# lucidrains/magvit2-pytorch

Hardware: NVIDIA H100
Metric: video-frames/sec tokenize+decode, 17x128x128 bf16 (higher is better)
Workload: dtype bf16

## Files before the change

### magvit2_pytorch_b200/csrc/tc_common.cuh

```cuda
#pragma once
#include "common.cuh"
#include <cuda.h>
#include <mutex>

namespace mv2 {


__device__ __forceinline__ uint32_t smem_u32(const void* p) { return (uint32_t)__cvta_generic_to_shared(p); }

__device__ __forceinline__ void mbar_init(uint32_t bar, uint32_t count) {
  asm volatile("mbarrier.init.shared::cta.b64 [%0], %1;" ::"r"(bar), "r"(count));
}
__device__ __forceinline__ void mbar_expect_tx(uint32_t bar, uint32_t bytes) {
  asm volatile("mbarrier.arrive.expect_tx.shared::cta.b64 _, [%0], %1;" ::"r"(bar), "r"(bytes) : "memory");
}
__device__ __forceinline__ void mbar_wait(uint32_t bar, uint32_t parity) {
  asm volatile(
      "{\n\t"
      ".reg .pred P1;\n\t"
      "WAIT_LOOP:\n\t"
      "mbarrier.try_wait.parity.shared::cta.b64 P1, [%0], %1, 0x989680;\n\t"
      "@P1 bra DONE;\n\t"
      "bra WAIT_LOOP;\n\t"
      "DONE:\n\t"
      "}" ::"r"(bar), "r"(parity) : "memory");
}
__device__ __forceinline__ void fence_barrier_init() { asm volatile("fence.mbarrier_init.release.cluster;" ::: "memory"); }
__device__ __forceinline__ void fence_proxy_async() { asm volatile("fence.proxy.async.shared::cta;" ::: "memory"); }

__device__ __forceinline__ void tma_load_5d(uint32_t dst, const CUtensorMap* map, uint32_t bar, int c0, int c1, int c2,
                                            int c3, int c4) {
  asm volatile(
      "cp.async.bulk.tensor.5d.shared::cluster.global.tile.mbarrier::complete_tx::bytes [%0], [%1, {%3, %4, %5, %6, %7}], [%2];"
      ::"r"(dst), "l"(map), "r"(bar), "r"(c0), "r"(c1), "r"(c2), "r"(c3), "r"(c4) : "memory");
}
__device__ __forceinline__ void tma_load_2d(uint32_t dst, const CUtensorMap* map, uint32_t bar, int c0, int c1) {
  asm volatile(
      "cp.async.bulk.tensor.2d.shared::cluster.global.tile.mbarrier::complete_tx::bytes [%0], [%1, {%3, %4}], [%2];"
      ::"r"(dst), "l"(map), "r"(bar), "r"(c0), "r"(c1) : "memory");
}
__device__ __forceinline__ void tma_load_3d(uint32_t dst, const CUtensorMap* map, uint32_t bar, int c0, int c1, int c2) {
  asm volatile(
      "cp.async.bulk.tensor.3d.shared::cluster.global.tile.mbarrier::complete_tx::bytes [%0], [%1, {%3, %4, %5}], [%2];"
      ::"r"(dst), "l"(map), "r"(bar), "r"(c0), "r"(c1), "r"(c2) : "memory");
}
__device__ __forceinline__ void tma_prefetch_desc(const CUtensorMap* map) {
  asm volatile("prefetch.tensormap [%0];" ::"l"(map) : "memory");
}

__device__ __forceinline__ void wgmma_fence() { asm volatile("wgmma.fence.sync.aligned;" ::: "memory"); }
__device__ __forceinline__ void wgmma_commit() { asm volatile("wgmma.commit_group.sync.aligned;" ::: "memory"); }
__device__ __forceinline__ void wgmma_wait_all() { asm volatile("wgmma.wait_group.sync.aligned 0;" ::: "memory"); }
template <int N> __device__ __forceinline__ void wgmma_bf16(float (&d)[N / 2], uint64_t da, uint64_t db, uint32_t scale_d);
template <> __device__ __forceinline__ void wgmma_bf16<32>(float (&d)[16], uint64_t da, uint64_t db, uint32_t scale_d) {
  asm volatile(
      "{\n\t.reg .pred p;\n\tsetp.ne.b32 p, %18, 0;\n\t"
      "wgmma.mma_async.sync.aligned.m64n32k16.f32.bf16.bf16 {%0, %1, %2, %3, %4, %5, %6, %7, %8, %9, %10, %11, %12, %13, %14, %15}, %16, %17, p, 1, 1, 0, 0;\n\t}"
      : "+f"(d[0]), "+f"(d[1]), "+f"(d[2]), "+f"(d[3]), "+f"(d[4]), "+f"(d[5]), "+f"(d[6]), "+f"(d[7]), "+f"(d[8]), "+f"(d[9]), "+f"(d[10]), "+f"(d[11]), "+f"(d[12]), "+f"(d[13]), "+f"(d[14]), "+f"(d[15])
      : "l"(da), "l"(db), "r"(scale_d));
}
template <> __device__ __forceinline__ void wgmma_bf16<64>(float (&d)[32], uint64_t da, uint64_t db, uint32_t scale_d) {
  asm volatile(
      "{\n\t.reg .pred p;\n\tsetp.ne.b32 p, %34, 0;\n\t"
      "wgmma.mma_async.sync.aligned.m64n64k16.f32.bf16.bf16 {%0, %1, %2, %3, %4, %5, %6, %7, %8, %9, %10, %11, %12, %13, %14, %15, %16, %17, %18, %19, %20, %21, %22, %23, %24, %25, %26, %27, %28, %29, %30, %31}, %32, %33, p, 1, 1, 0, 0;\n\t}"
      : "+f"(d[0]), "+f"(d[1]), "+f"(d[2]), "+f"(d[3]), "+f"(d[4]), "+f"(d[5]), "+f"(d[6]), "+f"(d[7]), "+f"(d[8]), "+f"(d[9]), "+f"(d[10]), "+f"(d[11]), "+f"(d[12]), "+f"(d[13]), "+f"(d[14]), "+f"(d[15]), "+f"(d[16]), "+f"(d[17]), "+f"(d[18]), "+f"(d[19]), "+f"(d[20]), "+f"(d[21]), "+f"(d[22]), "+f"(d[23]), "+f"(d[24]), "+f"(d[25]), "+f"(d[26]), "+f"(d[27]), "+f"(d[28]), "+f"(d[29]), "+f"(d[30]), "+f"(d[31])
      : "l"(da), "l"(db), "r"(scale_d));
}
template <> __device__ __forceinline__ void wgmma_bf16<128>(float (&d)[64], uint64_t da, uint64_t db, uint32_t scale_d) {
  asm volatile(
      "{\n\t.reg .pred p;\n\tsetp.ne.b32 p, %66, 0;\n\t"
      "wgmma.mma_async.sync.aligned.m64n128k16.f32.bf16.bf16 {%0, %1, %2, %3, %4, %5, %6, %7, %8, %9, %10, %11, %12, %13, %14, %15, %16, %17, %18, %19, %20, %21, %22, %23, %24, %25, %26, %27, %28, %29, %30, %31, %32, %33, %34, %35, %36, %37, %38, %39, %40, %41, %42, %43, %44, %45, %46, %47, %48, %49, %50, %51, %52, %53, %54, %55, %56, %57, %58, %59, %60, %61, %62, %63}, %64, %65, p, 1, 1, 0, 0;\n\t}"
      : "+f"(d[0]), "+f"(d[1]), "+f"(d[2]), "+f"(d[3]), "+f"(d[4]), "+f"(d[5]), "+f"(d[6]), "+f"(d[7]), "+f"(d[8]), "+f"(d[9]), "+f"(d[10]), "+f"(d[11]), "+f"(d[12]), "+f"(d[13]), "+f"(d[14]), "+f"(d[15]), "+f"(d[16]), "+f"(d[17]), "+f"(d[18]), "+f"(d[19]), "+f"(d[20]), "+f"(d[21]), "+f"(d[22]), "+f"(d[23]), "+f"(d[24]), "+f"(d[25]), "+f"(d[26]), "+f"(d[27]), "+f"(d[28]), "+f"(d[29]), "+f"(d[30]), "+f"(d[31]), "+f"(d[32]), "+f"(d[33]), "+f"(d[34]), "+f"(d[35]), "+f"(d[36]), "+f"(d[37]), "+f"(d[38]), "+f"(d[39]), "+f"(d[40]), "+f"(d[41]), "+f"(d[42]), "+f"(d[43]), "+f"(d[44]), "+f"(d[45]), "+f"(d[46]), "+f"(d[47]), "+f"(d[48]), "+f"(d[49]), "+f"(d[50]), "+f"(d[51]), "+f"(d[52]), "+f"(d[53]), "+f"(d[54]), "+f"(d[55]), "+f"(d[56]), "+f"(d[57]), "+f"(d[58]), "+f"(d[59]), "+f"(d[60]), "+f"(d[61]), "+f"(d[62]), "+f"(d[63])
      : "l"(da), "l"(db), "r"(scale_d));
}

__host__ __device__ __forceinline__ uint64_t gmma_desc_hi(uint32_t sbo, uint32_t row_bytes) {
  const uint64_t layout = row_bytes == 128 ? 1 : (row_bytes == 64 ? 2 : 3);
  return ((uint64_t)1 << 16) | ((uint64_t)(sbo >> 4) << 32) | (layout << 62);
}
__device__ __forceinline__ uint32_t desc_lo(uint32_t saddr) { return (saddr & 0x3FFFF) >> 4; }

template <int N> __device__ __forceinline__ void stage_acc(const float (&d)[N / 2], float* stg, int t) {
  const int r = 16 * (t >> 5) + ((t & 31) >> 2), c = 2 * (t & 3);
#pragma unroll
  for (int j = 0; j < N / 8; ++j) {
    *reinterpret_cast<float2*>(stg + r * (N + 4) + 8 * j + c) = make_float2(d[4 * j], d[4 * j + 1]);
    *reinterpret_cast<float2*>(stg + (r + 8) * (N + 4) + 8 * j + c) = make_float2(d[4 * j + 2], d[4 * j + 3]);
  }
}
__device__ __forceinline__ void load_row32(const float* src, int ncols, uint32_t (&r)[32]) {
#pragma unroll
  for (int g = 0; g < 8; ++g) {
    if (g * 4 >= ncols) break;
    const float4 v = *reinterpret_cast<const float4*>(src + 4 * g);
    r[4 * g] = __float_as_uint(v.x); r[4 * g + 1] = __float_as_uint(v.y);
    r[4 * g + 2] = __float_as_uint(v.z); r[4 * g + 3] = __float_as_uint(v.w);
  }
}
__device__ __forceinline__ void named_bar_sync(uint32_t id, uint32_t nthreads) {
  asm volatile("bar.sync %0, %1;" ::"r"(id), "r"(nthreads) : "memory");
}
__device__ __forceinline__ void mbar_arrive(uint32_t bar) {
  asm volatile("mbarrier.arrive.shared::cta.b64 _, [%0];" ::"r"(bar) : "memory");
}

__device__ __forceinline__ uint32_t pack_bf16x2(float a, float b) {
  __nv_bfloat162 v = __floats2bfloat162_rn(a, b);
  return *reinterpret_cast<uint32_t*>(&v);
}



struct TcEpi {
  const float* bias;
  const __nv_bfloat16* res;
  __nv_bfloat16* y;
  int act, shuffle, mode;
  int Co;
  int To, Ho, Wo;
  int out_cf;
  const float* oscale;
};

__device__ __forceinline__ void store8_bf16(__nv_bfloat16* dst, const float (&v)[8]) {
  uint4 o;
  o.x = pack_bf16x2(v[0], v[1]); o.y = pack_bf16x2(v[2], v[3]);
  o.z = pack_bf16x2(v[4], v[5]); o.w = pack_bf16x2(v[6], v[7]);
  *reinterpret_cast<uint4*>(dst) = o;
}

enum { EPI_PLAIN = 0, EPI_GEGLU = 1, EPI_SHUFFLE = 2, EPI_RAGGED = 3, EPI_PLAIN_RES = 4, EPI_FUSED_RU = 5, EPI_SHUFFLE_ST = 6,
       EPI_DOWN_SPACE = 7 };

__device__ __forceinline__ float ex2_approx(float x) {
  float y;
// ... 211 lines not shown
```

### magvit2_pytorch_b200/csrc/tc_conv.cu

```cuda
#include "common.cuh"
#include "tc_common.cuh"
#include <cuda.h>
#include <mutex>
#include <algorithm>
#include <string.h>

namespace mv2 {

constexpr int TC_MAX_TAPS = 64;
constexpr int TC_MAX_MAPS = 8;
constexpr int TC_BM = 128;

struct alignas(64) TcParams {
  CUtensorMap amap[TC_MAX_MAPS];
  CUtensorMap wmap;
  int8_t tap_map[TC_MAX_TAPS], tap_dt[TC_MAX_TAPS], tap_dh[TC_MAX_TAPS], tap_dw[TC_MAX_TAPS];
  int ntaps, kchunks, ci_pad, bk;
  int B, To, Ho, Wo, Co;
  int bt, bh, bw, tt, th, tw;
  int bn, stages;
  TcEpi epi;
};

template <int MODE, int BN>
__global__ void __launch_bounds__(384, 1) tc_conv_kernel(const __grid_constant__ TcParams p) {
  extern __shared__ uint8_t smem_raw[];
  const uint32_t smem_base = (smem_u32(smem_raw) + 1023u) & ~1023u;
  const int warp = threadIdx.x >> 5, lane = threadIdx.x & 31;
  const int bk = p.bk;
  const uint32_t row_bytes = bk * 2;
  const uint32_t a_bytes = TC_BM * row_bytes;
  const uint32_t b_bytes = BN * row_bytes;
  const uint32_t stage_bytes = a_bytes + b_bytes;
  const uint32_t bar_base = smem_base + p.stages * stage_bytes;
  const uint32_t full0 = bar_base, empty0 = bar_base + 8 * p.stages;
  const uint32_t sbias_u = (empty0 + 8 * p.stages + 15) & ~15u;
  float* sbias = reinterpret_cast<float*>(smem_raw + (sbias_u - smem_u32(smem_raw)));
  float* stg_all = sbias + BN;

  int tile = blockIdx.x;
  const int iw = tile % p.tw; tile /= p.tw;
  const int ih = tile % p.th; tile /= p.th;
  const int it = tile % p.tt; tile /= p.tt;
  const int b = tile;
  const int w0 = iw * p.bw, h0 = ih * p.bh, t0 = it * p.bt;
  const int n0 = blockIdx.y * BN;

  if (threadIdx.x == 0) {
    for (int s = 0; s < p.stages; ++s) {
      mbar_init(full0 + 8 * s, 1);
      mbar_init(empty0 + 8 * s, 8);
    }
    fence_barrier_init();
  }
  if (warp == 0 && lane == 0) {
    tma_prefetch_desc(&p.wmap);
    tma_prefetch_desc(&p.amap[0]);
  }
  if (warp >= 4)
    for (int i = threadIdx.x - 128; i < BN; i += 256) sbias[i] = (p.epi.bias && n0 + i < p.Co) ? p.epi.bias[n0 + i] : 0.f;
  __syncthreads();
  pdl_wait();
  pdl_launch_dependents();

  const int n_iters = p.ntaps * p.kchunks;
  if (warp == 0) {
    if (lane == 0) {
      uint32_t s = 0, ph = 0;
      int tap = 0, kc = 0;
      for (int i = 0; i < n_iters; ++i) {
        mbar_wait(empty0 + 8 * s, ph ^ 1);
        mbar_expect_tx(full0 + 8 * s, stage_bytes);
        const uint32_t sa = smem_base + s * stage_bytes;
        tma_load_5d(sa, &p.amap[p.tap_map[tap]], full0 + 8 * s, kc * bk, w0 + p.tap_dw[tap], h0 + p.tap_dh[tap],
                    t0 + p.tap_dt[tap], b);
        tma_load_2d(sa + a_bytes, &p.wmap, full0 + 8 * s, tap * p.ci_pad + kc * bk, n0);
        if (++kc == p.kchunks) { kc = 0; ++tap; }
        if (++s == (uint32_t)p.stages) { s = 0; ph ^= 1; }
      }
    }
  } else if (warp >= 4) {
    const int wg = (warp - 4) >> 2, t = threadIdx.x & 127;
    const uint64_t d_hi = gmma_desc_hi(8 * row_bytes, row_bytes);
    const int ksteps = bk >> 4;
    const uint32_t stage16 = stage_bytes >> 4, a16 = a_bytes >> 4, wg16 = (uint32_t)wg * ((64 * row_bytes) >> 4);
    uint32_t s = 0, ph = 0, lo = desc_lo(smem_base);
    float acc[BN / 2];
    for (int i = 0; i < n_iters; ++i) {
      mbar_wait(full0 + 8 * s, ph);
      wgmma_fence();
      const uint64_t ad = d_hi | (uint64_t)(lo + wg16);
      const uint64_t bd = d_hi | (uint64_t)(lo + a16);
      wgmma_bf16<BN>(acc, ad, bd, i > 0 ? 1u : 0u);
      if (ksteps > 1) wgmma_bf16<BN>(acc, ad + 2, bd + 2, 1u);
      if (ksteps > 2) {
        wgmma_bf16<BN>(acc, ad + 4, bd + 4, 1u);
        wgmma_bf16<BN>(acc, ad + 6, bd + 6, 1u);
      }
      wgmma_commit();
      wgmma_wait_all();
      __syncwarp();
      if (lane == 0) mbar_arrive(empty0 + 8 * s);
      if (++s == (uint32_t)p.stages) { s = 0; ph ^= 1; lo = desc_lo(smem_base); } else { lo += stage16; }
    }
    float* stg = stg_all + wg * 64 * (BN + 4);
    stage_acc<BN>(acc, stg, t);
    named_bar_sync(1 + wg, 128);
    const int wq = warp & 3;
    const int sub = 2 * wg + (wq & 1), half = wq >> 1;
    const int row = sub * 32 + lane;
    const int lw = row % p.bw, lh = (row / p.bw) % p.bh, lt = row / (p.bw * p.bh);
    const int wo = w0 + lw, ho = h0 + lh, to = t0 + lt;
    const bool row_ok = wo < p.Wo && ho < p.Ho && to < p.To;
    const int64_t row_base = ((((int64_t)b * p.To + to) * p.Ho + ho) * p.Wo + wo) * p.Co;
    const float* srow = stg + (row - 64 * wg) * (BN + 4);
    for (int c0 = half * 32; c0 < BN; c0 += 64) {
      uint32_t r[32];
      load_row32(srow + c0, 32, r);
      if (row_ok) epi_chunk32<MODE>(p.epi, r, 32, n0 + c0, sbias + c0, b, to, ho, wo, row_base);
    }
  }
}

#define MV2_TC_BN(M) {tc_conv_kernel<M, 32>, tc_conv_kernel<M, 64>, tc_conv_kernel<M, 128>}
static void (*const g_tc_kernels[3][3])(TcParams) = {MV2_TC_BN(EPI_RAGGED), MV2_TC_BN(EPI_GEGLU), MV2_TC_BN(EPI_SHUFFLE)};
#undef MV2_TC_BN

}

using namespace mv2;

extern "C" {

int mv2_tc_conv_supported(const mv2_tc_conv_args* a) {
  if (!a) return 0;
  if (a->Ci % 16 != 0) return 0;
  if (a->kt * a->kh * a->kw > TC_MAX_TAPS) return 0;
  if (a->st < 1 || a->st > 2 || a->sh < 1 || a->sh > 2 || a->sw < 1 || a->sw > 2) return 0;
  if (a->shuffle != MV2_SHUFFLE_NONE && ((a->shuffle == MV2_SHUFFLE_SPACE ? a->Co / 4 : a->Co / 2) % 8 != 0)) return 0;
  if (a->res && a->Co % 8 != 0) return 0;
  if (a->epi_mode == 1 && (a->Co % 32 != 0 || a->shuffle != MV2_SHUFFLE_NONE || a->res)) return 0;
  if (a->epi_mode == 2 && (!a->res || a->shuffle != MV2_SHUFFLE_NONE)) return 0;
  if (a->epi_mode < 0 || a->epi_mode > 2) return 0;
  if (a->out_layout != 0) return 0;
  if (a->oscale && (a->epi_mode != 0 || a->shuffle != MV2_SHUFFLE_NONE)) return 0;
  return 1;
}

int mv2_tc_conv_forward(const mv2_tc_conv_args* a, void* stream) {
  MV2_CHECK_ARG(a && a->x && a->w && a->y);
  if (!mv2_tc_conv_supported(a)) { set_error("mv2_tc_conv_forward: unsupported shape (Ci=%d Co=%d)", a->Ci, a->Co); return MV2_E_UNSUPPORTED; }

  TcParams p;
  memset(&p, 0, sizeof(p));
  const int bk = (a->Ci % 64 == 0) ? 64 : ((a->Ci % 32 == 0) ? 32 : 16);
  const CUtensorMapSwizzle swz = swizzle_of_row(bk * 2);
  p.bk = bk;
  p.ci_pad = a->Ci;
  p.kchunks = a->Ci / bk;
  p.B = a->B; p.To = a->To; p.Ho = a->Ho; p.Wo = a->Wo; p.Co = a->Co;
  p.bw = std::min(128, pow2_ceil(a->Wo));
  p.bh = std::min(128 / p.bw, pow2_ceil(a->Ho));
  p.bt = 128 / (p.bw * p.bh);
  p.tw = ceil_div(a->Wo, p.bw); p.th = ceil_div(a->Ho, p.bh); p.tt = ceil_div(a->To, p.bt);
  const int bn = a->Co <= 32 ? 32 : (a->Co <= 64 ? 64 : 128);
  const int row_bytes = bk * 2;
  p.bn = bn;
  const int stage_bytes = TC_BM * row_bytes + bn * row_bytes;
  MV2_CHECK_ARG((TC_BM * row_bytes) % 1024 == 0 && (bn * row_bytes) % 1024 == 0);
  const int stg_bytes = 2 * 64 * (bn + 4) * 4;
  int stages = (200 * 1024 - stg_bytes) / stage_bytes;
  stages = std::max(2, std::min(stages, 8));
  stages = std::max(1, std::min(stages, a->kt * a->kh * a->kw * (a->Ci / bk)));
  p.stages = stages;
  p.epi = tc_epi_of(a);

  const int st = a->st, sh = a->sh, sw = a->sw;
  const int nmaps = st * sh * sw;
  MV2_CHECK_ARG(nmaps <= TC_MAX_MAPS);
  const int64_t C = a->Ci, W = a->Wi, H = a->Hi, T = a->Ti;
  for (int pt = 0; pt < st; ++pt)
    for (int ph = 0; ph < sh; ++ph)
      for (int pw = 0; pw < sw; ++pw) {
        const int id = (pt * sh + ph) * sw + pw;
        const int64_t nW = (W - pw + sw - 1) / sw, nH = (H - ph + sh - 1) / sh, nT = (T - pt + st - 1) / st;
        if (nW <= 0 || nH <= 0 || nT <= 0) { set_error("empty stride phase (dimension smaller than stride)"); return MV2_E_UNSUPPORTED; }
        const cuuint64_t dims[5] = {(cuuint64_t)C, (cuuint64_t)nW, (cuuint64_t)nH, (cuuint64_t)nT, (cuuint64_t)a->B};
// ... 46 lines not shown
```

### magvit2_pytorch_b200/csrc/tc_slab.cu

```cuda
#include "common.cuh"
#include "tc_common.cuh"
#include <cuda.h>
#include <algorithm>
#include <mutex>
#include <map>
#include <vector>
#include <string.h>

namespace mv2 {

struct alignas(64) SlabParams {
  CUtensorMap amap;
  CUtensorMap wmap;
  CUtensorMap wmap2;
  int kt, kh, kw, pt, ph, pw;
  int st;
  int Ci, kchunks, row_bytes;
  int B, T, H, W, Co;
  int mw, pitch, slab_h, slab_bytes, slab_stride;
  int bn, n_tiles_n, tiles_w, tiles_h, total_tiles;
  int slab_stages, w_stages;
  int tpw;
  TcEpi epi;
  CUtensorMap w1map;
// ... 14 lines not shown
  const int full_slots = p.B * n_full;
  if (slot < full_slots) { b = slot / n_full; t = n_cheap + slot - b * n_full; }
  else { const int r = slot - full_slots; const int level = r / p.B; b = r - level * p.B; t = n_cheap - 1 - level; }
}
__host__ __device__ __forceinline__ int slab_tile_of_cta(const SlabParams& p, int k, int cta, int grid) {
  const int tile = k * grid + ((k & 1) ? grid - 1 - cta : cta);
  return tile < p.total_tiles ? tile : -1;
}
__device__ __forceinline__ int slab_tile_of(const SlabParams& p, int k) { return slab_tile_of_cta(p, k, blockIdx.x, gridDim.x); }

struct TileCoord { int b, t, h0, w0, n0; };
__host__ __device__ __forceinline__ TileCoord decode_tile(const SlabParams& p, int tile) {
  TileCoord c;
  const int nt = tile % p.n_tiles_n; tile /= p.n_tiles_n;
  const int tw = tile % p.tiles_w; tile /= p.tiles_w;
  const int th = tile % p.tiles_h; tile /= p.tiles_h;
  slab_frame_of(p, tile, c.b, c.t);
  c.h0 = th * 16;
  c.w0 = tw * 8 * p.mw;
  c.n0 = nt * p.bn;
  return c;
}

struct SlabSmem { uint32_t sbias, stage0, lpart, accstg, hbuf, w1buf, end; };
__host__ __device__ __forceinline__ SlabSmem slab_smem_layout(const SlabParams& p, uint32_t bar0, bool fused) {
  SlabSmem m;
  m.sbias = (bar0 + 8 * (2 * p.slab_stages + 2 * p.w_stages + 1) + 15) & ~15u;
  m.stage0 = m.sbias + (uint32_t)(p.n_tiles_n * p.bn) * 4 * (fused ? 3 : 1);
  m.lpart = m.stage0 + (fused ? 0 : 8 * 2048);
  m.accstg = m.lpart + (fused ? 2048 : 0);
  m.hbuf = m.accstg + 2u * p.mw * 64 * (p.bn + 4) * 4;
  if (fused) m.hbuf = (m.hbuf + 1023u) & ~1023u;
  m.w1buf = m.hbuf + (fused ? (uint32_t)p.h_stride : 0);
  m.end = m.w1buf + (fused ? (uint32_t)(p.kchunks * p.bn * p.row_bytes) : 0);
  return m;
}

template <int MODE, int BN>
__global__ void __launch_bounds__(384, 1) tc_slab_kernel(const __grid_constant__ SlabParams p) {
  constexpr int MWMAX = 128 / BN;
  extern __shared__ uint8_t smem_raw[];
  const uint32_t smem_base = (smem_u32(smem_raw) + 1023u) & ~1023u;
  const int warp = threadIdx.x >> 5, lane = threadIdx.x & 31;
  const uint32_t row_bytes = p.row_bytes;
  const uint32_t bk = row_bytes >> 1;
  const uint32_t w_tile = p.bn * row_bytes;
  const uint32_t w_bytes = w_tile * p.tpw;
  const uint32_t slab0 = smem_base;
  const uint32_t wst0 = smem_base + p.slab_stages * p.slab_stride;
  const uint32_t bar0 = wst0 + p.w_stages * w_bytes;
  const uint32_t slab_full = bar0, slab_empty = slab_full + 8 * p.slab_stages;
  const uint32_t w_full = slab_empty + 8 * p.slab_stages, w_empty = w_full + 8 * p.w_stages;
  const uint32_t w1_full = w_empty + 8 * p.w_stages;
  const SlabSmem L = slab_smem_layout(p, bar0, MODE == EPI_FUSED_RU);
  auto gen = [&](uint32_t u) { return smem_raw + (u - smem_u32(smem_raw)); };
  float* sbias = reinterpret_cast<float*>(gen(L.sbias));
  const uint32_t nbias = (uint32_t)(p.n_tiles_n * p.bn);
  const uint32_t stage0 = L.stage0;

  if (threadIdx.x == 0) {
    for (int s = 0; s < p.slab_stages; ++s) { mbar_init(slab_full + 8 * s, 1); mbar_init(slab_empty + 8 * s, 8); }
    for (int s = 0; s < p.w_stages; ++s) { mbar_init(w_full + 8 * s, 1); mbar_init(w_empty + 8 * s, 8); }
    mbar_init(w1_full, 1);
    fence_barrier_init();
  }
  if (warp == 0 && lane == 0) { tma_prefetch_desc(&p.amap); if (MODE == EPI_DOWN_SPACE) tma_prefetch_desc(&p.amap_odd); }
  if (warp == 2 && lane == 0) { tma_prefetch_desc(&p.wmap); tma_prefetch_desc(&p.wmap2); }
  if (MODE == EPI_FUSED_RU && warp == 3 && lane == 0) tma_prefetch_desc(&p.w1map);
  if (warp >= 4) {
    const int nb = p.n_tiles_n * p.bn;
    for (int i = threadIdx.x - 128; i < nb; i += 256) sbias[i] = (p.epi.bias && i < p.Co) ? p.epi.bias[i] : 0.f;
    if (MODE == EPI_FUSED_RU)
      for (int i = threadIdx.x - 128; i < nb; i += 256) {
        sbias[nb + i] = (p.bias1 && i < p.Co) ? p.bias1[i] : 0.f;
        sbias[2 * nb + i] = i < p.Co ? p.se_wk[i] : 0.f;
      }
  }
  __syncthreads();
  pdl_wait();
  pdl_launch_dependents();

  const int taps2d = p.kh * p.kw;

  if (warp == 0) {
    if (MODE == EPI_DOWN_SPACE) {
      if (lane == 0) {
        uint32_t s = 0, ph = 0;
        for (int tk = 0, tile; (tile = slab_tile_of(p, tk)) >= 0; ++tk) {
          const TileCoord c = decode_tile(p, tile);
          for (int kc = 0; kc < p.kchunks; ++kc) {
            mbar_wait(slab_empty + 8 * s, ph ^ 1);
            mbar_expect_tx(slab_full + 8 * s, p.slab_bytes);
            tma_load_5d(slab0 + s * p.slab_stride, &p.amap_odd, slab_full + 8 * s, kc * bk, c.w0 - 1, c.h0 - 1, c.t, c.b);
            tma_load_5d(slab0 + s * p.slab_stride + p.dn_e_off, &p.amap, slab_full + 8 * s, kc * bk, c.w0 - 1, c.h0, c.t, c.b);
            if (++s == (uint32_t)p.slab_stages) { s = 0; ph ^= 1; }
          }
        }
      }
    } else
    if (lane == 0) {
      uint32_t s = 0, ph = 0;
      for (int tk = 0, tile; (tile = slab_tile_of(p, tk)) >= 0; ++tk) {
        const TileCoord c = decode_tile(p, tile);
        const int dt0 = max(0, p.pt - c.t * p.st);
        for (int dt = dt0; dt < p.kt; ++dt)
          for (int kc = 0; kc < p.kchunks; ++kc) {
            mbar_wait(slab_empty + 8 * s, ph ^ 1);
            mbar_expect_tx(slab_full + 8 * s, p.slab_bytes);
            tma_load_5d(slab0 + s * p.slab_stride, &p.amap, slab_full + 8 * s, kc * bk, c.w0 - p.pw, c.h0 - p.ph,
                        c.t * p.st + dt - p.pt, c.b);
            if (++s == (uint32_t)p.slab_stages) { s = 0; ph ^= 1; }
          }
      }
    }
  } else if (warp == 2) {
    if (MODE == EPI_DOWN_SPACE) {
      if (lane == 0) {
        uint32_t s = 0, ph = 0;
        const int C2 = p.Ci;
        for (int tk = 0, tile; (tile = slab_tile_of(p, tk)) >= 0; ++tk) {
          const TileCoord c = decode_tile(p, tile);
          for (int kc = 0; kc < p.kchunks; ++kc)
            for (int tap = kc < p.dn_lower ? 1 : 0; tap < 6; tap += kc < p.dn_lower ? 2 : 1) {
              mbar_wait(w_empty + 8 * s, ph ^ 1);
              mbar_expect_tx(w_full + 8 * s, w_tile);
              tma_load_2d(wst0 + s * w_bytes, &p.wmap2, w_full + 8 * s, tap * C2 + kc * (int)bk, c.n0);
              if (++s == (uint32_t)p.w_stages) { s = 0; ph ^= 1; }
            }
        }
      }
    } else
    if (lane == 0) {
      uint32_t s = 0, ph = 0;
      for (int tk = 0, tile; (tile = slab_tile_of(p, tk)) >= 0; ++tk) {
        const TileCoord c = decode_tile(p, tile);
        const int dt0 = max(0, p.pt - c.t * p.st);
        for (int dt = dt0; dt < p.kt; ++dt)
          for (int kc = 0; kc < p.kchunks; ++kc)
            for (int tp = 0; tp < taps2d; tp += p.tpw) {
              mbar_wait(w_empty + 8 * s, ph ^ 1);
              mbar_expect_tx(w_full + 8 * s, w_bytes);
              if (p.tpw == 1) tma_load_2d(wst0 + s * w_bytes, &p.wmap2, w_full + 8 * s, (dt * taps2d + tp) * p.Ci + kc * bk, c.n0);
              else tma_load_3d(wst0 + s * w_bytes, &p.wmap, w_full + 8 * s, kc * bk, c.n0, dt * taps2d + tp);
              if (++s == (uint32_t)p.w_stages) { s = 0; ph ^= 1; }
            }
      }
    }
  } else if (warp == 3) {
    if (MODE == EPI_FUSED_RU && lane == 0) {
      mbar_expect_tx(w1_full, (uint32_t)p.kchunks * w_tile);
      for (int kc2 = 0; kc2 < p.kchunks; ++kc2) tma_load_2d(L.w1buf + kc2 * w_tile, &p.w1map, w1_full, kc2 * (int)bk, 0);
    }
  } else if (warp >= 4) {
    const int wg = (warp - 4) >> 2, wq = warp & 3, tid = threadIdx.x & 127;
    const int sub = 2 * wg + (wq & 1), half = wq >> 1, ew = sub + 4 * half;
    const int row = sub * 32 + lane;
    const int lh = row >> 3, lw = row & 7;
    float* stg = reinterpret_cast<float*>(gen(L.accstg)) + (size_t)wg * p.mw * 64 * (BN + 4);
    const uint32_t wg_bar = 5 + wg;
    const uint32_t sbo = (uint32_t)p.pitch * row_bytes;
    const uint64_t a_hi = gmma_desc_hi(sbo, row_bytes);
    const uint64_t b_hi = gmma_desc_hi(8 * row_bytes, row_bytes);
    const bool k4 = bk == 64;
    const uint32_t a_row = row_bytes >> 4;
    const uint32_t a_wg = (uint32_t)wg * 8 * (sbo >> 4);
    const uint32_t a_next_dh = (uint32_t)(p.pitch - p.kw + 1) * a_row;
    const uint32_t a_mtile = 8 * a_row;
    const uint32_t w_tile16 = w_tile >> 4, w_stage16 = w_bytes >> 4;
    const uint32_t b_lo0 = desc_lo(wst0);
    uint32_t s_idx = 0, s_par = 0;
    uint32_t w_idx = 0, w_par = 0, b_lo = b_lo0;
    uint32_t ecount = 0;
    if (MODE == EPI_FUSED_RU) mbar_wait(w1_full, 0);
    float acc[MWMAX][BN / 2];
    for (int tk = 0, tile; (tile = slab_tile_of(p, tk)) >= 0; ++tk) {
      const TileCoord c = decode_tile(p, tile);
      uint32_t accum = 0;
      if (MODE == EPI_DOWN_SPACE) {
        for (int kc = 0; kc < p.kchunks; ++kc) {
          mbar_wait(slab_full + 8 * s_idx, s_par);
          const uint32_t a_base = desc_lo(slab0 + s_idx * p.slab_stride) + a_wg;
          const int t0 = kc < p.dn_lower ? 1 : 0, tstep = kc < p.dn_lower ? 2 : 1;
          for (int tap = t0; tap < 6; tap += tstep) {
            mbar_wait(w_full + 8 * w_idx, w_par);
            wgmma_fence();
            const uint64_t bd = b_hi | (uint64_t)b_lo;
#pragma unroll
            for (int j = 0; j < MWMAX; ++j) {
              if (j >= p.mw) break;
              const uint64_t ad = a_hi | (uint64_t)(a_base + (uint32_t)p.dn_aoff[tap] + j * a_mtile);
              wgmma_bf16<BN>(acc[j], ad, bd, accum);
              wgmma_bf16<BN>(acc[j], ad + 2, bd + 2, 1u);
              wgmma_bf16<BN>(acc[j], ad + 4, bd + 4, 1u);
              wgmma_bf16<BN>(acc[j], ad + 6, bd + 6, 1u);
            }
            wgmma_commit();
            wgmma_wait_all();
            __syncwarp();
            if (lane == 0) mbar_arrive(w_empty + 8 * w_idx);
            accum = 1;
            if (++w_idx == (uint32_t)p.w_stages) { w_idx = 0; w_par ^= 1; b_lo = b_lo0; } else { b_lo += w_stage16; }
          }
          if (lane == 0) mbar_arrive(slab_empty + 8 * s_idx);
          if (++s_idx == (uint32_t)p.slab_stages) { s_idx = 0; s_par ^= 1; }
        }
      } else {
        const int dt0 = max(0, p.pt - c.t * p.st);
        for (int dt = dt0; dt < p.kt; ++dt)
          for (int kc = 0; kc < p.kchunks; ++kc) {
            mbar_wait(slab_full + 8 * s_idx, s_par);
            uint32_t a_lo = desc_lo(slab0 + s_idx * p.slab_stride) + a_wg;
            int dw = 0;
            for (int tp0 = 0; tp0 < taps2d; tp0 += p.tpw) {
              mbar_wait(w_full + 8 * w_idx, w_par);
              wgmma_fence();
              uint32_t b_cur = b_lo;
              for (int u = 0; u < p.tpw; ++u) {
                const uint64_t bd = b_hi | (uint64_t)b_cur;
#pragma unroll
                for (int j = 0; j < MWMAX; ++j) {
                  if (j >= p.mw) break;
                  const uint64_t ad = a_hi | (uint64_t)(a_lo + j * a_mtile);
                  wgmma_bf16<BN>(acc[j], ad, bd, accum);
                  wgmma_bf16<BN>(acc[j], ad + 2, bd + 2, 1u);
                  if (k4) {
                    wgmma_bf16<BN>(acc[j], ad + 4, bd + 4, 1u);
                    wgmma_bf16<BN>(acc[j], ad + 6, bd + 6, 1u);
                  }
                }
                accum = 1;
                b_cur += w_tile16;
                if (++dw == p.kw) { dw = 0; a_lo += a_next_dh; } else { a_lo += a_row; }
              }
              wgmma_commit();
              wgmma_wait_all();
              __syncwarp();
              if (lane == 0) mbar_arrive(w_empty + 8 * w_idx);
              if (++w_idx == (uint32_t)p.w_stages) { w_idx = 0; w_par ^= 1; b_lo = b_lo0; } else { b_lo += w_stage16; }
            }
            if (lane == 0) mbar_arrive(slab_empty + 8 * s_idx);
            if (++s_idx == (uint32_t)p.slab_stages) { s_idx = 0; s_par ^= 1; }
          }
      }
      named_bar_sync(wg_bar, 128);
#pragma unroll
      for (int j = 0; j < MWMAX; ++j) {
        if (j >= p.mw) break;
        stage_acc<BN>(acc[j], stg + j * 64 * (BN + 4), tid);
      }
      named_bar_sync(wg_bar, 128);
      const int h = c.h0 + lh;
      if (MODE == EPI_FUSED_RU) {
        const float* sb1 = sbias + nbias;
        const float* swk = sbias + 2 * nbias;
        float* lpart = reinterpret_cast<float*>(gen(L.lpart));
        const int64_t kstride = (int64_t)p.W * p.Co;
        const uint32_t wsw = (lane >> 1) & 3;
        const int rl = lane >> 2, piece = lane & 3;
        const int h20 = c.h0 + sub * 4;
        const int recs_per_frame = p.tiles_h * p.tiles_w * 4;
        float* rec = p.se_ws + ((int64_t)(c.b * p.T + c.t) * recs_per_frame + ((c.h0 >> 4) * p.tiles_w + c.w0 / (8 * p.mw)) * 4 + sub) * (p.Co + 2);
        float run_m = -INFINITY, run_s = 0.f, run_acc[2][8];
#pragma unroll
        for (int q = 0; q < 2; ++q)
#pragma unroll
          for (int i = 0; i < 8; ++i) run_acc[q][i] = 0.f;
        const uint64_t h_hi = gmma_desc_hi(1024, 128);
        const uint32_t h_lo = desc_lo(L.hbuf) + (uint32_t)wg * ((64 * 128) >> 4), w1_lo = desc_lo(L.w1buf);
        for (int j = 0; j < p.mw; ++j) {
          const float* srow = stg + (j * 64 + row - 64 * wg) * (BN + 4);
          const uint32_t stg2 = smem_u32(stg + (j * 64 + (sub & 1) * 32) * (BN + 4)) + (uint32_t)half * 2048;
          const uint32_t wr = stg2 + lane * 64, rd = stg2 + rl * 64;
          const uint32_t hb = L.hbuf + (uint32_t)row * 128;
          for (int c0 = half * 32; c0 < p.bn; c0 += 64) {
            uint32_t r[32], pk[16];
            load_row32(srow + c0, 32, r);
            epi_pack32_t<MV2_ACT_ELU>(r, sbias + c0, pk);
            const uint32_t hrow = hb + (uint32_t)(c0 >> 6) * 16384;
            const uint32_t p0 = (uint32_t)(c0 & 63) >> 3;
#pragma unroll
            for (int g = 0; g < 4; ++g)
              asm volatile("st.shared.v4.b32 [%0], {%1, %2, %3, %4};" ::"r"(hrow + (((p0 + g) ^ ((uint32_t)row & 7u)) << 4)),
                           "r"(pk[4 * g]), "r"(pk[4 * g + 1]), "r"(pk[4 * g + 2]), "r"(pk[4 * g + 3]) : "memory");
          }
          fence_proxy_async();
          named_bar_sync(wg_bar, 128);
          wgmma_fence();
          for (int kc2 = 0; kc2 < p.kchunks; ++kc2) {
            const uint64_t ad = h_hi | (uint64_t)(h_lo + kc2 * (16384 >> 4)), bd = h_hi | (uint64_t)(w1_lo + kc2 * (w_tile >> 4));
            wgmma_bf16<BN>(acc[0], ad, bd, kc2 > 0 ? 1u : 0u);
            wgmma_bf16<BN>(acc[0], ad + 2, bd + 2, 1u);
            wgmma_bf16<BN>(acc[0], ad + 4, bd + 4, 1u);
            wgmma_bf16<BN>(acc[0], ad + 6, bd + 6, 1u);
          }
          wgmma_commit();
          wgmma_wait_all();
          stage_acc<BN>(acc[0], stg + j * 64 * (BN + 4), tid);
          named_bar_sync(wg_bar, 128);
          const int w = c.w0 + 8 * j + lw;
          const bool row_ok = h < p.H && w < p.W;
          uint32_t pk2[2][16];
          float lp = 0.f;
#pragma unroll
          for (int q = 0; q < 2; ++q) {
            const int c0 = half * 32 + 64 * q;
            if (c0 < p.bn) {
              uint32_t r[32];
              load_row32(srow + c0, 32, r);
              epi_pack32_t<MV2_ACT_ELU>(r, sb1 + c0, pk2[q]);
#pragma unroll
              for (int i = 0; i < 16; i += 2) {
                const float4 wv = *reinterpret_cast<const float4*>(swk + c0 + 2 * i);
                lp = fmaf(__uint_as_float(pk2[q][i] << 16), wv.x, lp);
                lp = fmaf(__uint_as_float(pk2[q][i] & 0xffff0000u), wv.y, lp);
                lp = fmaf(__uint_as_float(pk2[q][i + 1] << 16), wv.z, lp);
                lp = fmaf(__uint_as_float(pk2[q][i + 1] & 0xffff0000u), wv.w, lp);
              }
            }
          }
          float* lpb = lpart + (ecount & 1u) * 256;
          ++ecount;
          lpb[ew * 32 + lane] = lp;
          asm volatile("bar.sync %0, 64;" ::"r"(1 + sub) : "memory");
          float lg = lpb[sub * 32 + lane] + lpb[(sub + 4) * 32 + lane] + p.se_bk;
          lg = row_ok ? lg : -INFINITY;
          const float mx = warp_max(lg);
// ... 451 lines not shown
```

Baseline: 4443.

## Keep one wgmma group in flight and rebalance registers across warp roles

The consumer loops in the TC conv and slab conv kernels now issue the next stage's wgmma group before waiting on the previous one (wait_group 1), so stage buffers are released one step later and tensor-core work overlaps the next mbarrier wait. The slab kernel's per-tile nested loops are flattened into issue/release lambdas with separate release counters for weight and slab stages. A 'hold' mode handles when deferred release is safe given the stage counts. Producer warps shrink their register budget with setmaxnreg.dec and consumer warpgroups grow theirs with setmaxnreg.inc. The risks are buffer-release ordering bugs (tied to the stage-count conditions) and register-limit constraints.

Result: no change. 4470, median of 6 (+0.6%).

```diff
diff --git a/magvit2_pytorch_b200/csrc/tc_common.cuh b/magvit2_pytorch_b200/csrc/tc_common.cuh
--- a/magvit2_pytorch_b200/csrc/tc_common.cuh
+++ b/magvit2_pytorch_b200/csrc/tc_common.cuh
@@ -51,6 +51,9 @@
 __device__ __forceinline__ void wgmma_fence() { asm volatile("wgmma.fence.sync.aligned;" ::: "memory"); }
 __device__ __forceinline__ void wgmma_commit() { asm volatile("wgmma.commit_group.sync.aligned;" ::: "memory"); }
 __device__ __forceinline__ void wgmma_wait_all() { asm volatile("wgmma.wait_group.sync.aligned 0;" ::: "memory"); }
+template <int N> __device__ __forceinline__ void wgmma_wait() { asm volatile("wgmma.wait_group.sync.aligned %0;" ::"n"(N) : "memory"); }
+template <int R> __device__ __forceinline__ void setmaxnreg_dec() { asm volatile("setmaxnreg.dec.sync.aligned.u32 %0;" ::"n"(R)); }
+template <int R> __device__ __forceinline__ void setmaxnreg_inc() { asm volatile("setmaxnreg.inc.sync.aligned.u32 %0;" ::"n"(R)); }
 template <int N> __device__ __forceinline__ void wgmma_bf16(float (&d)[N / 2], uint64_t da, uint64_t db, uint32_t scale_d);
 template <> __device__ __forceinline__ void wgmma_bf16<32>(float (&d)[16], uint64_t da, uint64_t db, uint32_t scale_d) {
   asm volatile(
diff --git a/magvit2_pytorch_b200/csrc/tc_conv.cu b/magvit2_pytorch_b200/csrc/tc_conv.cu
--- a/magvit2_pytorch_b200/csrc/tc_conv.cu
+++ b/magvit2_pytorch_b200/csrc/tc_conv.cu
@@ -85,24 +85,31 @@
     const int ksteps = bk >> 4;
     const uint32_t stage16 = stage_bytes >> 4, a16 = a_bytes >> 4, wg16 = (uint32_t)wg * ((64 * row_bytes) >> 4);
     uint32_t s = 0, ph = 0, lo = desc_lo(smem_base);
+    uint32_t s_rel = 0;
     float acc[BN / 2];
-    for (int i = 0; i < n_iters; ++i) {
+    auto issue_stage = [&](uint32_t accum) {
       mbar_wait(full0 + 8 * s, ph);
       wgmma_fence();
       const uint64_t ad = d_hi | (uint64_t)(lo + wg16);
       const uint64_t bd = d_hi | (uint64_t)(lo + a16);
-      wgmma_bf16<BN>(acc, ad, bd, i > 0 ? 1u : 0u);
+      wgmma_bf16<BN>(acc, ad, bd, accum);
       if (ksteps > 1) wgmma_bf16<BN>(acc, ad + 2, bd + 2, 1u);
       if (ksteps > 2) {
         wgmma_bf16<BN>(acc, ad + 4, bd + 4, 1u);
         wgmma_bf16<BN>(acc, ad + 6, bd + 6, 1u);
       }
       wgmma_commit();
-      wgmma_wait_all();
+      if (++s == (uint32_t)p.stages) { s = 0; ph ^= 1; lo = desc_lo(smem_base); } else { lo += stage16; }
+    };
+    issue_stage(0u);
+    for (int i = 1; i < n_iters; ++i) {
+      issue_stage(1u);
+      wgmma_wait<1>();
       __syncwarp();
-      if (lane == 0) mbar_arrive(empty0 + 8 * s);
-      if (++s == (uint32_t)p.stages) { s = 0; ph ^= 1; lo = desc_lo(smem_base); } else { lo += stage16; }
-    }
+      if (lane == 0) mbar_arrive(empty0 + 8 * s_rel);
+      if (++s_rel == (uint32_t)p.stages) s_rel = 0;
+    }
+    wgmma_wait<0>();
     float* stg = stg_all + wg * 64 * (BN + 4);
     stage_acc<BN>(acc, stg, t);
     named_bar_sync(1 + wg, 128);
diff --git a/magvit2_pytorch_b200/csrc/tc_slab.cu b/magvit2_pytorch_b200/csrc/tc_slab.cu
--- a/magvit2_pytorch_b200/csrc/tc_slab.cu
+++ b/magvit2_pytorch_b200/csrc/tc_slab.cu
@@ -120,76 +120,80 @@
 
   const int taps2d = p.kh * p.kw;
 
-  if (warp == 0) {
-    if (MODE == EPI_DOWN_SPACE) {
+  if (warp < 4) {
+    setmaxnreg_dec<40>();
+    if (warp == 0) {
+      if (MODE == EPI_DOWN_SPACE) {
+        if (lane == 0) {
+          uint32_t s = 0, ph = 0;
+          for (int tk = 0, tile; (tile = slab_tile_of(p, tk)) >= 0; ++tk) {
+            const TileCoord c = decode_tile(p, tile);
+            for (int kc = 0; kc < p.kchunks; ++kc) {
+              mbar_wait(slab_empty + 8 * s, ph ^ 1);
+              mbar_expect_tx(slab_full + 8 * s, p.slab_bytes);
+              tma_load_5d(slab0 + s * p.slab_stride, &p.amap_odd, slab_full + 8 * s, kc * bk, c.w0 - 1, c.h0 - 1, c.t, c.b);
+              tma_load_5d(slab0 + s * p.slab_stride + p.dn_e_off, &p.amap, slab_full + 8 * s, kc * bk, c.w0 - 1, c.h0, c.t, c.b);
+              if (++s == (uint32_t)p.slab_stages) { s = 0; ph ^= 1; }
+            }
+          }
+        }
+      } else
       if (lane == 0) {
         uint32_t s = 0, ph = 0;
         for (int tk = 0, tile; (tile = slab_tile_of(p, tk)) >= 0; ++tk) {
           const TileCoord c = decode_tile(p, tile);
-          for (int kc = 0; kc < p.kchunks; ++kc) {
-            mbar_wait(slab_empty + 8 * s, ph ^ 1);
-            mbar_expect_tx(slab_full + 8 * s, p.slab_bytes);
-            tma_load_5d(slab0 + s * p.slab_stride, &p.amap_odd, slab_full + 8 * s, kc * bk, c.w0 - 1, c.h0 - 1, c.t, c.b);
-            tma_load_5d(slab0 + s * p.slab_stride + p.dn_e_off, &p.amap, slab_full + 8 * s, kc * bk, c.w0 - 1, c.h0, c.t, c.b);
-            if (++s == (uint32_t)p.slab_stages) { s = 0; ph ^= 1; }
-          }
+          const int dt0 = max(0, p.pt - c.t * p.st);
+          for (int dt = dt0; dt < p.kt; ++dt)
+            for (int kc = 0; kc < p.kchunks; ++kc) {
+              mbar_wait(slab_empty + 8 * s, ph ^ 1);
+              mbar_expect_tx(slab_full + 8 * s, p.slab_bytes);
+              tma_load_5d(slab0 + s * p.slab_stride, &p.amap, slab_full + 8 * s, kc * bk, c.w0 - p.pw, c.h0 - p.ph,
+                          c.t * p.st + dt - p.pt, c.b);
+              if (++s == (uint32_t)p.slab_stages) { s = 0; ph ^= 1; }
+            }
         }
       }
-    } else
-    if (lane == 0) {
-      uint32_t s = 0, ph = 0;
-      for (int tk = 0, tile; (tile = slab_tile_of(p, tk)) >= 0; ++tk) {
-        const TileCoord c = decode_tile(p, tile);
-        const int dt0 = max(0, p.pt - c.t * p.st);
-        for (int dt = dt0; dt < p.kt; ++dt)
-          for (int kc = 0; kc < p.kchunks; ++kc) {
-            mbar_wait(slab_empty + 8 * s, ph ^ 1);
-            mbar_expect_tx(slab_full + 8 * s, p.slab_bytes);
-            tma_load_5d(slab0 + s * p.slab_stride, &p.amap, slab_full + 8 * s, kc * bk, c.w0 - p.pw, c.h0 - p.ph,
-                        c.t * p.st + dt - p.pt, c.b);
-            if (++s == (uint32_t)p.slab_stages) { s = 0; ph ^= 1; }
-          }
+    } else if (warp == 2) {
+      if (MODE == EPI_DOWN_SPACE) {
+        if (lane == 0) {
+          uint32_t s = 0, ph = 0;
+          const int C2 = p.Ci;
+          for (int tk = 0, tile; (tile = slab_tile_of(p, tk)) >= 0; ++tk) {
+            const TileCoord c = decode_tile(p, tile);
+            for (int kc = 0; kc < p.kchunks; ++kc)
+              for (int tap = kc < p.dn_lower ? 1 : 0; tap < 6; tap += kc < p.dn_lower ? 2 : 1) {
+                mbar_wait(w_empty + 8 * s, ph ^ 1);
+                mbar_expect_tx(w_full + 8 * s, w_tile);
+                tma_load_2d(wst0 + s * w_bytes, &p.wmap2, w_full + 8 * s, tap * C2 + kc * (int)bk, c.n0);
+                if (++s == (uint32_t)p.w_stages) { s = 0; ph ^= 1; }
+              }
+          }
+        }
+      } else
+      if (lane == 0) {
+        uint32_t s = 0, ph = 0;
+        for (int tk = 0, tile; (tile = slab_tile_of(p, tk)) >= 0; ++tk) {
+          const TileCoord c = decode_tile(p, tile);
+          const int dt0 = max(0, p.pt - c.t * p.st);
+          for (int dt = dt0; dt < p.kt; ++dt)
+            for (int kc = 0; kc < p.kchunks; ++kc)
+              for (int tp = 0; tp < taps2d; tp += p.tpw) {
+                mbar_wait(w_empty + 8 * s, ph ^ 1);
+                mbar_expect_tx(w_full + 8 * s, w_bytes);
+                if (p.tpw == 1) tma_load_2d(wst0 + s * w_bytes, &p.wmap2, w_full + 8 * s, (dt * taps2d + tp) * p.Ci + kc * bk, c.n0);
+                else tma_load_3d(wst0 + s * w_bytes, &p.wmap, w_full + 8 * s, kc * bk, c.n0, dt * taps2d + tp);
+                if (++s == (uint32_t)p.w_stages) { s = 0; ph ^= 1; }
+              }
+        }
+      }
+    } else if (warp == 3) {
+      if (MODE == EPI_FUSED_RU && lane == 0) {
+        mbar_expect_tx(w1_full, (uint32_t)p.kchunks * w_tile);
+        for (int kc2 = 0; kc2 < p.kchunks; ++kc2) tma_load_2d(L.w1buf + kc2 * w_tile, &p.w1map, w1_full, kc2 * (int)bk, 0);
       }
     }
-  } else if (warp == 2) {
-    if (MODE == EPI_DOWN_SPACE) {
-      if (lane == 0) {
-        uint32_t s = 0, ph = 0;
-        const int C2 = p.Ci;
-        for (int tk = 0, tile; (tile = slab_tile_of(p, tk)) >= 0; ++tk) {
-          const TileCoord c = decode_tile(p, tile);
-          for (int kc = 0; kc < p.kchunks; ++kc)
-            for (int tap = kc < p.dn_lower ? 1 : 0; tap < 6; tap += kc < p.dn_lower ? 2 : 1) {
-              mbar_wait(w_empty + 8 * s, ph ^ 1);
-              mbar_expect_tx(w_full + 8 * s, w_tile);
-              tma_load_2d(wst0 + s * w_bytes, &p.wmap2, w_full + 8 * s, tap * C2 + kc * (int)bk, c.n0);
-              if (++s == (uint32_t)p.w_stages) { s = 0; ph ^= 1; }
-            }
-        }
-      }
-    } else
-    if (lane == 0) {
-      uint32_t s = 0, ph = 0;
-      for (int tk = 0, tile; (tile = slab_tile_of(p, tk)) >= 0; ++tk) {
-        const TileCoord c = decode_tile(p, tile);
-        const int dt0 = max(0, p.pt - c.t * p.st);
-        for (int dt = dt0; dt < p.kt; ++dt)
-          for (int kc = 0; kc < p.kchunks; ++kc)
-            for (int tp = 0; tp < taps2d; tp += p.tpw) {
-              mbar_wait(w_empty + 8 * s, ph ^ 1);
-              mbar_expect_tx(w_full + 8 * s, w_bytes);
-              if (p.tpw == 1) tma_load_2d(wst0 + s * w_bytes, &p.wmap2, w_full + 8 * s, (dt * taps2d + tp) * p.Ci + kc * bk, c.n0);
-              else tma_load_3d(wst0 + s * w_bytes, &p.wmap, w_full + 8 * s, kc * bk, c.n0, dt * taps2d + tp);
-              if (++s == (uint32_t)p.w_stages) { s = 0; ph ^= 1; }
-            }
-      }
-    }
-  } else if (warp == 3) {
-    if (MODE == EPI_FUSED_RU && lane == 0) {
-      mbar_expect_tx(w1_full, (uint32_t)p.kchunks * w_tile);
-      for (int kc2 = 0; kc2 < p.kchunks; ++kc2) tma_load_2d(L.w1buf + kc2 * w_tile, &p.w1map, w1_full, kc2 * (int)bk, 0);
-    }
-  } else if (warp >= 4) {
+  } else {
+    setmaxnreg_inc<232>();
     const int wg = (warp - 4) >> 2, wq = warp & 3, tid = threadIdx.x & 127;
     const int sub = 2 * wg + (wq & 1), half = wq >> 1, ew = sub + 4 * half;
     const int row = sub * 32 + lane;
@@ -208,78 +212,102 @@
     const uint32_t b_lo0 = desc_lo(wst0);
     uint32_t s_idx = 0, s_par = 0;
     uint32_t w_idx = 0, w_par = 0, b_lo = b_lo0;
+    int tp = 0, dw = 0, kc_i = 0, tap_i = MODE == EPI_DOWN_SPACE && p.dn_lower > 0 ? 1 : 0;
+    uint32_t a_lo = 0;
+    uint32_t w_rel = 0, s_rel = 0;
+    int rel_k = 0, rel_kc = 0;
+    int rel_n = MODE == EPI_DOWN_SPACE ? (p.dn_lower > 0 ? 3 : 6) : taps2d / p.tpw;
+    const bool hold = p.w_stages > 2 && (p.slab_stages > 2 || MODE == EPI_DOWN_SPACE || taps2d / p.tpw > 1);
+    uint32_t accum = 0;
     uint32_t ecount = 0;
     if (MODE == EPI_FUSED_RU) mbar_wait(w1_full, 0);
     float acc[MWMAX][BN / 2];
+    auto issue_stage = [&]() {
+      if (MODE == EPI_DOWN_SPACE) {
+        const bool lower = kc_i < p.dn_lower;
+        if (tap_i == (lower ? 1 : 0)) {
+          mbar_wait(slab_full + 8 * s_idx, s_par);
+          a_lo = desc_lo(slab0 + s_idx * p.slab_stride) + a_wg;
+        }
+        mbar_wait(w_full + 8 * w_idx, w_par);
+        wgmma_fence();
+        const uint64_t bd = b_hi | (uint64_t)b_lo;
+#pragma unroll
+        for (int j = 0; j < MWMAX; ++j) {
+          if (j >= p.mw) break;
+          const uint64_t ad = a_hi | (uint64_t)(a_lo + (uint32_t)p.dn_aoff[tap_i] + j * a_mtile);
+          wgmma_bf16<BN>(acc[j], ad, bd, accum);
+          wgmma_bf16<BN>(acc[j], ad + 2, bd + 2, 1u);
+          wgmma_bf16<BN>(acc[j], ad + 4, bd + 4, 1u);
+          wgmma_bf16<BN>(acc[j], ad + 6, bd + 6, 1u);
+        }
+        wgmma_commit();
+        accum = 1;
+        if ((tap_i += lower ? 2 : 1) >= 6) {
+          if (++kc_i == p.kchunks) kc_i = 0;
+          tap_i = kc_i < p.dn_lower ? 1 : 0;
+          if (++s_idx == (uint32_t)p.slab_stages) { s_idx = 0; s_par ^= 1; }
+        }
+      } else {
+        if (tp == 0) {
+          mbar_wait(slab_full + 8 * s_idx, s_par);
+          a_lo = desc_lo(slab0 + s_idx * p.slab_stride) + a_wg;
+        }
+        mbar_wait(w_full + 8 * w_idx, w_par);
+        wgmma_fence();
+        uint32_t b_cur = b_lo;
+        for (int u = 0; u < p.tpw; ++u) {
+          const uint64_t bd = b_hi | (uint64_t)b_cur;
+#pragma unroll
+          for (int j = 0; j < MWMAX; ++j) {
+            if (j >= p.mw) break;
+            const uint64_t ad = a_hi | (uint64_t)(a_lo + j * a_mtile);
+            wgmma_bf16<BN>(acc[j], ad, bd, accum);
+            wgmma_bf16<BN>(acc[j], ad + 2, bd + 2, 1u);
+            if (k4) {
+              wgmma_bf16<BN>(acc[j], ad + 4, bd + 4, 1u);
+              wgmma_bf16<BN>(acc[j], ad + 6, bd + 6, 1u);
+            }
+          }
+          accum = 1;
+          b_cur += w_tile16;
+          if (++dw == p.kw) { dw = 0; a_lo += a_next_dh; } else { a_lo += a_row; }
+        }
+        wgmma_commit();
+        if ((tp += p.tpw) == taps2d) {
+          tp = 0;
+          if (++s_idx == (uint32_t)p.slab_stages) { s_idx = 0; s_par ^= 1; }
+        }
+      }
+      if (++w_idx == (uint32_t)p.w_stages) { w_idx = 0; w_par ^= 1; b_lo = b_lo0; } else { b_lo += w_stage16; }
+    };
+    auto release_stage = [&]() {
+      __syncwarp();
+      if (lane == 0) mbar_arrive(w_empty + 8 * w_rel);
+      if (++w_rel == (uint32_t)p.w_stages) w_rel = 0;
+      if (++rel_k == rel_n) {
+        if (lane == 0) mbar_arrive(slab_empty + 8 * s_rel);
+        if (++s_rel == (uint32_t)p.slab_stages) s_rel = 0;
+        rel_k = 0;
+        if (MODE == EPI_DOWN_SPACE) {
+          if (++rel_kc == p.kchunks) rel_kc = 0;
+          rel_n = rel_kc < p.dn_lower ? 3 : 6;
+        }
+      }
+    };
     for (int tk = 0, tile; (tile = slab_tile_of(p, tk)) >= 0; ++tk) {
       const TileCoord c = decode_tile(p, tile);
-      uint32_t accum = 0;
-      if (MODE == EPI_DOWN_SPACE) {
-        for (int kc = 0; kc < p.kchunks; ++kc) {
-          mbar_wait(slab_full + 8 * s_idx, s_par);
-          const uint32_t a_base = desc_lo(slab0 + s_idx * p.slab_stride) + a_wg;
-          const int t0 = kc < p.dn_lower ? 1 : 0, tstep = kc < p.dn_lower ? 2 : 1;
-          for (int tap = t0; tap < 6; tap += tstep) {
-            mbar_wait(w_full + 8 * w_idx, w_par);
-            wgmma_fence();
-            const uint64_t bd = b_hi | (uint64_t)b_lo;
-#pragma unroll
-            for (int j = 0; j < MWMAX; ++j) {
-              if (j >= p.mw) break;
-              const uint64_t ad = a_hi | (uint64_t)(a_base + (uint32_t)p.dn_aoff[tap] + j * a_mtile);
-              wgmma_bf16<BN>(acc[j], ad, bd, accum);
-              wgmma_bf16<BN>(acc[j], ad + 2, bd + 2, 1u);
-              wgmma_bf16<BN>(acc[j], ad + 4, bd + 4, 1u);
-              wgmma_bf16<BN>(acc[j], ad + 6, bd + 6, 1u);
-            }
-            wgmma_commit();
-            wgmma_wait_all();
-            __syncwarp();
-            if (lane == 0) mbar_arrive(w_empty + 8 * w_idx);
-            accum = 1;
-            if (++w_idx == (uint32_t)p.w_stages) { w_idx = 0; w_par ^= 1; b_lo = b_lo0; } else { b_lo += w_stage16; }
-          }
-          if (lane == 0) mbar_arrive(slab_empty + 8 * s_idx);
-          if (++s_idx == (uint32_t)p.slab_stages) { s_idx = 0; s_par ^= 1; }
-        }
-      } else {
-        const int dt0 = max(0, p.pt - c.t * p.st);
-        for (int dt = dt0; dt < p.kt; ++dt)
-          for (int kc = 0; kc < p.kchunks; ++kc) {
-            mbar_wait(slab_full + 8 * s_idx, s_par);
-            uint32_t a_lo = desc_lo(slab0 + s_idx * p.slab_stride) + a_wg;
-            int dw = 0;
-            for (int tp0 = 0; tp0 < taps2d; tp0 += p.tpw) {
-              mbar_wait(w_full + 8 * w_idx, w_par);
-              wgmma_fence();
-              uint32_t b_cur = b_lo;
-              for (int u = 0; u < p.tpw; ++u) {
-                const uint64_t bd = b_hi | (uint64_t)b_cur;
-#pragma unroll
-                for (int j = 0; j < MWMAX; ++j) {
-                  if (j >= p.mw) break;
-                  const uint64_t ad = a_hi | (uint64_t)(a_lo + j * a_mtile);
-                  wgmma_bf16<BN>(acc[j], ad, bd, accum);
-                  wgmma_bf16<BN>(acc[j], ad + 2, bd + 2, 1u);
-                  if (k4) {
-                    wgmma_bf16<BN>(acc[j], ad + 4, bd + 4, 1u);
-                    wgmma_bf16<BN>(acc[j], ad + 6, bd + 6, 1u);
-                  }
-                }
-                accum = 1;
-                b_cur += w_tile16;
-                if (++dw == p.kw) { dw = 0; a_lo += a_next_dh; } else { a_lo += a_row; }
-              }
-              wgmma_commit();
-              wgmma_wait_all();
-              __syncwarp();
-              if (lane == 0) mbar_arrive(w_empty + 8 * w_idx);
-              if (++w_idx == (uint32_t)p.w_stages) { w_idx = 0; w_par ^= 1; b_lo = b_lo0; } else { b_lo += w_stage16; }
-            }
-            if (lane == 0) mbar_arrive(slab_empty + 8 * s_idx);
-            if (++s_idx == (uint32_t)p.slab_stages) { s_idx = 0; s_par ^= 1; }
-          }
+      const int n_stages = MODE == EPI_DOWN_SPACE ? p.dn_lower * 3 + (p.kchunks - p.dn_lower) * 6
+                                                  : (p.kt - max(0, p.pt - c.t * p.st)) * p.kchunks * (taps2d / p.tpw);
+      accum = 0;
+      for (int k = 0; k < n_stages; ++k) {
+        issue_stage();
+        if (!hold) wgmma_commit();
+        wgmma_wait<1>();
+        if (k > 0 || !hold) release_stage();
       }
+      wgmma_wait<0>();
+      if (hold) release_stage();
       named_bar_sync(wg_bar, 128);
 #pragma unroll
       for (int j = 0; j < MWMAX; ++j) {
```
